# zpelgrims/pota

Hardware: AMD Instinct MI355X
Metric: bidir redistribution Msamples/s at 4K, double-gauss 50mm (higher is better)
Workload: dtype f64

## Files before the change

### include/lentil_hip.h

```cpp
#ifndef LENTIL_HIP_H
#define LENTIL_HIP_H

#include <stddef.h>
#include <stdint.h>

#ifdef __cplusplus
extern "C" {
#endif

#define LENTIL_ABI_VERSION 1

#define LENTIL_OK 0
#define LENTIL_ERR_INVALID (-1)
#define LENTIL_ERR_HIP (-2)
#define LENTIL_ERR_UNSUPPORTED (-3)
#define LENTIL_ERR_NOMEM (-4)

#define LENTIL_THINLENS 0
#define LENTIL_POLYNOMIAL_OPTICS 1
#define LENTIL_UNIT_MM 0
#define LENTIL_UNIT_CM 1
#define LENTIL_UNIT_DM 2
#define LENTIL_UNIT_M 3
#define LENTIL_FILTER_GAUSSIAN 0
// ... 267 lines not shown
  uint64_t first_ray;
  const float *in;
  float *out;
  int32_t *tries;
  double lambda;
  float exposure;
  uint32_t rng_seed;
  uint32_t flags;
} lentil_camera_ray_batch;
int lentil_hip_camera_rays(lentil_hip_ctx *ctx, const lentil_camera_ray_batch *batch);

int lentil_hip_test_y0_intersection(lentil_hip_ctx *ctx, uint64_t n, const double *sensor_shift, double lambda,
                                    double *distance, double *sensor, double *out);
int lentil_hip_test_lt_sample_aperture(lentil_hip_ctx *ctx, uint64_t n, const double *scene,
                                       const double *ap, double lambda, double *sensor,
                                       double *out, double *transmittance);
int lentil_hip_test_trace_bw_po(lentil_hip_ctx *ctx, uint64_t n, const double *target,
                                const int32_t *px, const int32_t *py, const int32_t *attempt,
                                double *sensor_xy, int32_t *ok);
int lentil_hip_test_aperture_sample(lentil_hip_ctx *ctx, uint64_t n, const uint32_t *a,
                                    const uint32_t *b, double *xy);
int lentil_hip_test_xor128_jump(const uint32_t in[4], uint64_t k, uint32_t out[4]);
int lentil_hip_debug_scan_bands(const lentil_params *params, float out[8]);
enum {
  LENTIL_SCAN_DMA2 = 1,
  LENTIL_SCAN_DMA = 2,
  LENTIL_SCAN_DMA_MULTI = 3,
  LENTIL_SCAN_UNIFORM = 4,
  LENTIL_SCAN_UNIFORM_MULTI = 5,
  LENTIL_SCAN_RUNS = 6,
  LENTIL_SCAN_RAGGED = 7
};
int lentil_hip_debug_last_scan(lentil_hip_ctx *ctx, uint32_t out[4]);

#ifdef __cplusplus
}
#endif
#endif
```

### pota_amd/capi.py

```python
import ctypes as C
import os

import numpy as np

from . import _abi

_PKG = os.path.dirname(os.path.abspath(__file__))
LIB_PATH = os.environ.get("LENTIL_HIP_LIB") or os.path.join(_PKG, "liblentil_hip.so")

EXPORTS = [
    "lentil_hip_abi_version", "lentil_hip_create", "lentil_hip_destroy", "lentil_hip_last_error", "lentil_hip_last_redo_note",
    "lentil_hip_set_params", "lentil_hip_set_lens", "lentil_hip_set_bokeh", "lentil_hip_alloc_frame", "lentil_hip_set_camera_motion", "lentil_hip_set_camera_shutter",
    "lentil_hip_upload_visits", "lentil_hip_bind_visits", "lentil_hip_clear_frame",
    "lentil_hip_redistribute", "lentil_hip_resolve", "lentil_hip_sync", "lentil_hip_download_aov",
    "lentil_hip_download_accum", "lentil_hip_download_records", "lentil_hip_accum_buffer", "lentil_hip_stream",
    "lentil_hip_set_closest_exchange", "lentil_hip_zkey_buffer", "lentil_hip_closest_gather",
    "lentil_hip_touched_rows", "lentil_hip_merge_rows", "lentil_hip_resolve_rows",
    "lentil_hip_pack_rows", "lentil_hip_merge_packed_rows", "lentil_hip_compact_rows", "lentil_hip_merge_sparse",
    "lentil_hip_get_counters", "lentil_hip_last_timing", "lentil_hip_last_launches", "lentil_hip_set_draw_log",
    "lentil_hip_batch_model_stats", "lentil_hip_process_stats", "lentil_hip_process_stall_notes", "lentil_hip_set_async", "lentil_hip_pass_totals", "lentil_hip_set_occlusion_probe", "lentil_hip_probe_stats", "lentil_hip_debug_batch_estimate", "lentil_hip_box_probe",
    "lentil_hip_lens_jit_status", "lentil_hip_lens_jit_wait", "lentil_hip_debug_lens_jit_source", "lentil_hip_debug_lens_jit_compile",
    "lentil_hip_download_draw_log", "lentil_hip_test_lt_sample_aperture",
    "lentil_hip_test_trace_bw_po", "lentil_hip_test_aperture_sample", "lentil_hip_debug_scan_bands", "lentil_hip_debug_last_scan",
    "lentil_hip_lens_is_compiled", "lentil_hip_set_lens_mode",
    "lentil_hip_focus_search", "lentil_hip_test_y0_intersection", "lentil_hip_camera_rays",
    "lentil_hip_set_xor128_state", "lentil_hip_get_xor128_state", "lentil_hip_tl_chroma_stats", "lentil_hip_test_xor128_jump",
    "lentil_hip_host_alloc", "lentil_hip_host_free", "lentil_hip_visits_begin", "lentil_hip_visits_append",
    "lentil_hip_visits_wait", "lentil_hip_visits_end",
    "lentil_hip_comm_unique_id", "lentil_hip_comm_init", "lentil_hip_comm_destroy", "lentil_hip_allreduce",
    "lentil_hip_exchange_bands", "lentil_hip_exchange_stats", "lentil_hip_exchange_counts", "lentil_hip_degenerate_stats", "lentil_hip_streams_concurrent",
    "lentil_hip_alloc_crypto", "lentil_hip_upload_crypto", "lentil_hip_bind_crypto", "lentil_hip_download_crypto",
    "lentil_hip_download_crypto_table", "lentil_hip_visits_begin_crypto", "lentil_hip_visits_append_crypto",
]

SCAN_DMA2, SCAN_DMA, SCAN_DMA_MULTI, SCAN_UNIFORM, SCAN_UNIFORM_MULTI, SCAN_RUNS, SCAN_RAGGED = range(1, 8)
SCAN_NAMES = {SCAN_DMA2: "dma2", SCAN_DMA: "dma", SCAN_DMA_MULTI: "dma_multi", SCAN_UNIFORM: "uniform",
              SCAN_UNIFORM_MULTI: "uniform_multi", SCAN_RUNS: "runs", SCAN_RAGGED: "ragged"}

_lib = None


def process_stats():
    lib = load_library()
    n = (C.c_uint64 * 4)()
    rc = lib.lentil_hip_process_stats(n)
    if rc:
        raise RuntimeError("lentil_hip_process_stats: %d" % rc)
    return tuple(int(x) for x in n)


def process_stall_notes():
    lib = load_library()
    buf = C.create_string_buffer(1 << 14)
    lib.lentil_hip_process_stall_notes(buf, 1 << 14)
    return buf.value.decode(errors="replace")

# ... 47 lines not shown
        "lentil_hip_last_error": (C.c_char_p, [vp]),
        "lentil_hip_last_redo_note": (C.c_char_p, [vp]),
        "lentil_hip_set_params": (i, [vp, C.POINTER(_abi.Params)]),
        "lentil_hip_set_lens": (i, [vp, C.POINTER(_abi.LensTable)]),
        "lentil_hip_set_bokeh": (i, [vp, C.POINTER(_abi.BokehTable)]),
        "lentil_hip_alloc_frame": (i, [vp, u32, vp]),
        "lentil_hip_set_camera_motion": (i, [vp, u32, vp]),
        "lentil_hip_set_camera_shutter": (i, [vp, C.c_float, C.c_float]),
        "lentil_hip_upload_visits": (i, [vp, C.POINTER(_abi.Visits)]),
        "lentil_hip_bind_visits": (i, [vp, C.POINTER(_abi.Visits)]),
        "lentil_hip_clear_frame": (i, [vp]),
        "lentil_hip_redistribute": (i, [vp]),
        "lentil_hip_resolve": (i, [vp]),
        "lentil_hip_sync": (i, [vp]),
        "lentil_hip_download_aov": (i, [vp, u32, vp]),
        "lentil_hip_download_accum": (i, [vp, u32, vp, vp]),
        "lentil_hip_download_records": (i, [vp, vp, u64, C.POINTER(u32)]),
        "lentil_hip_accum_buffer": (i, [vp, C.POINTER(vp), C.POINTER(u64)]),
        "lentil_hip_stream": (i, [vp, C.POINTER(vp)]),
        "lentil_hip_set_closest_exchange": (i, [vp, i, u32]),
        "lentil_hip_zkey_buffer": (i, [vp, C.POINTER(vp), C.POINTER(u64)]),
        "lentil_hip_closest_gather": (i, [vp]),
        "lentil_hip_touched_rows": (i, [vp, C.POINTER(C.c_int32), C.POINTER(C.c_int32)]),
        "lentil_hip_merge_rows": (i, [vp, u32, u32, vp, vp]),
        "lentil_hip_pack_rows": (i, [vp, u32, u32, vp]),
        "lentil_hip_merge_packed_rows": (i, [vp, u32, u32, vp, vp]),
        "lentil_hip_compact_rows": (i, [vp, u32, u32, vp, vp, vp, u32, C.POINTER(u32)]),
        "lentil_hip_merge_sparse": (i, [vp, u32, u32, u32, vp, vp, vp]),
        "lentil_hip_resolve_rows": (i, [vp, u32, u32]),
        "lentil_hip_get_counters": (i, [vp, C.POINTER(_abi.Counters)]),
        "lentil_hip_last_timing": (i, [vp, C.POINTER(C.c_float)]),
        "lentil_hip_last_launches": (i, [vp, C.POINTER(C.c_uint32)]),
        "lentil_hip_debug_last_scan": (i, [vp, C.POINTER(C.c_uint32)]),
        "lentil_hip_batch_model_stats": (i, [vp, C.POINTER(C.c_uint64)]),
        "lentil_hip_process_stats": (i, [C.POINTER(C.c_uint64)]),
        "lentil_hip_process_stall_notes": (i, [C.c_char_p, C.c_uint64]),
        "lentil_hip_set_async": (i, [vp, i]),
        "lentil_hip_set_occlusion_probe": (i, [vp, vp, vp, vp]),
        "lentil_hip_probe_stats": (i, [vp, C.POINTER(C.c_uint64)]),
        "lentil_hip_pass_totals": (i, [vp, C.POINTER(_abi.PassTotals), i]),
        "lentil_hip_box_probe": (i, [vp, C.POINTER(C.c_double)]),
        "lentil_hip_lens_jit_status": (i, [vp, C.POINTER(C.c_int), C.POINTER(C.c_double)]),
        "lentil_hip_lens_jit_wait": (i, [vp, C.c_double]),
        "lentil_hip_debug_lens_jit_compile": (i, [vp, i, C.c_char_p, C.c_uint64, C.POINTER(C.c_uint64), C.c_char_p, C.c_uint64,
                                                  C.POINTER(C.c_double), C.POINTER(C.c_uint64)]),
        "lentil_hip_debug_lens_jit_source": (i, [vp, C.c_char_p, C.c_uint64, C.POINTER(C.c_uint64)]),
        "lentil_hip_debug_batch_estimate": (i, [vp, C.c_uint64, vp, C.c_uint32, vp]),
        "lentil_hip_alloc_crypto": (i, [vp, u32, u32]),
        "lentil_hip_upload_crypto": (i, [vp, C.POINTER(_abi.CryptoVisits)]),
        "lentil_hip_bind_crypto": (i, [vp, C.POINTER(_abi.CryptoVisits)]),
        "lentil_hip_download_crypto": (i, [vp, u32, u32, vp, vp]),
        "lentil_hip_visits_begin_crypto": (i, [vp, u32]),
        "lentil_hip_visits_append_crypto": (i, [vp, C.POINTER(_abi.Visits), C.POINTER(_abi.CryptoVisits), C.POINTER(u64)]),
        "lentil_hip_download_crypto_table": (i, [vp, u32, C.POINTER(u32), vp, vp, vp]),
        "lentil_hip_set_draw_log": (i, [vp, u64]),
        "lentil_hip_download_draw_log": (i, [vp, vp, u64, C.POINTER(u64)]),
        "lentil_hip_test_lt_sample_aperture": (i, [vp, u64, vp, vp, C.c_double, vp, vp, vp]),
        "lentil_hip_test_trace_bw_po": (i, [vp, u64, vp, vp, vp, vp, vp, vp]),
        "lentil_hip_test_aperture_sample": (i, [vp, u64, vp, vp, vp]),
        "lentil_hip_lens_is_compiled": (i, [vp]),
        "lentil_hip_set_lens_mode": (i, [vp, i]),
        "lentil_hip_focus_search": (i, [vp, C.c_double, C.c_double, C.POINTER(C.c_double)]),
        "lentil_hip_camera_rays": (i, [vp, C.POINTER(_abi.CameraRayBatch)]),
        "lentil_hip_set_xor128_state": (i, [vp, C.POINTER(C.c_uint32)]),
        "lentil_hip_get_xor128_state": (i, [vp, C.POINTER(C.c_uint32)]),
        "lentil_hip_tl_chroma_stats": (i, [vp, C.POINTER(u64), C.POINTER(u64), C.POINTER(u64)]),
# ... 385 lines not shown

    def set_occlusion_probe(self, fn, user=None, camera_to_world=None):
        self._probe_keep = (np.ascontiguousarray(camera_to_world, np.float32) if camera_to_world is not None else None)
        self._chk(self.lib.lentil_hip_set_occlusion_probe(self.h, fn, user, self._probe_keep.ctypes.data if self._probe_keep is not None else None))

    def probe_stats(self):
        n = (C.c_uint64 * 3)()
        self._chk(self.lib.lentil_hip_probe_stats(self.h, n))
        return tuple(int(x) for x in n)

    def set_async(self, on):
        self._chk(self.lib.lentil_hip_set_async(self.h, 1 if on else 0))

    def pass_totals(self, reset=False):
        t = _abi.PassTotals()
        self._chk(self.lib.lentil_hip_pass_totals(self.h, C.byref(t), 1 if reset else 0))
        return t

    def last_timing(self):
        ms = (C.c_float * 3)()
        self._chk(self.lib.lentil_hip_last_timing(self.h, ms))
        return float(ms[0]), float(ms[1]), float(ms[2])

    def last_launches(self):
        n = (C.c_uint32 * 2)()
        self._chk(self.lib.lentil_hip_last_launches(self.h, n))
        return int(n[0]), int(n[1])

    def last_scan(self):
        n = (C.c_uint32 * 4)()
        self._chk(self.lib.lentil_hip_debug_last_scan(self.h, n))
        return tuple(int(x) for x in n)

    def lens_jit_status(self):
        st, sec = C.c_int(0), C.c_double(0.0)
        self._chk(self.lib.lentil_hip_lens_jit_status(self.h, C.byref(st), C.byref(sec)))
        return int(st.value), float(sec.value)

    def lens_jit_wait(self, timeout_seconds=0.0):
        self._chk(self.lib.lentil_hip_lens_jit_wait(self.h, float(timeout_seconds)))

    def lens_jit_source(self):
        n = C.c_uint64(0)
        self._chk(self.lib.lentil_hip_debug_lens_jit_source(self.h, None, 0, C.byref(n)))
        buf = C.create_string_buffer(int(n.value) + 1)
        self._chk(self.lib.lentil_hip_debug_lens_jit_source(self.h, buf, int(n.value) + 1, None))
        return buf.value.decode()

    def box_probe(self):
        p = (C.c_double * 6)()
        self._chk(self.lib.lentil_hip_box_probe(self.h, p))
        return {"fp64_mul_add_tflops": round(p[0], 2), "shader_clock_mhz_under_fp64": round(p[1], 1), "copy_gbs": round(p[2], 1),
                "read_gbs": round(p[3], 1), "gpu_max_hw_queues": int(p[4]), "compute_units": int(p[5])}

    def batch_model_stats(self):
        n = (C.c_uint64 * 4)()
        self._chk(self.lib.lentil_hip_batch_model_stats(self.h, n))
        return tuple(int(x) for x in n)

    def debug_batch_estimate(self, cs_xyz, samples):
        import numpy as np
        cs = np.ascontiguousarray(cs_xyz, np.float32)
        out = np.zeros((cs.shape[0], 4), np.float32)
        self._chk(self.lib.lentil_hip_debug_batch_estimate(self.h, cs.shape[0], cs.ctypes.data, int(samples), out.ctypes.data))
        return out

# ... 64 lines not shown
```

### pota_amd/csrc/lentil_hip.hip

```cpp
#include <hip/hip_runtime.h>
#include <hip/hip_ext.h>

#include <algorithm>
#include <atomic>
#include <chrono>
#include <cmath>
#include <cstdio>
#include <cstdlib>
#include <cstring>
#include <deque>
#include <mutex>
#include <new>
#include <string>
#include <vector>

#include "lentil_kernels.h"
#include "lentil_closest_replay.h"
#include "lentil_tl_chroma_mgpu.h"
#include "lentil_lens_jit.h"
#include "lentil_camera_rays.h"
#include "generated/embedded_sources.inc"

#define LENTIL_API extern "C" __attribute__((visibility("default")))

// ... 3858 lines not shown
  ms[0] = ms[1] = ms[2] = 0.f;
  HIP_TRY(ctx, hipSetDevice(ctx->device));
  HIP_TRY(ctx, hipStreamSynchronize(ctx->stream));
  if (ctx->timed_draw) {
    HIP_TRY(ctx, hipEventElapsedTime(&ms[0], ctx->ev[0], ctx->ev[1]));
    HIP_TRY(ctx, hipEventElapsedTime(&ms[1], ctx->ev[1], ctx->ev[2]));
    if (ctx->scan_kernel_timed) {
      float k = 0.f;
      if (hipEventElapsedTime(&k, ctx->ev_scan_k[0], ctx->ev_scan_k[1]) == hipSuccess && k > 0.f && k <= ms[0]) {
        ms[1] += ms[0] - k;
        ms[0] = k;
      }
    }
  }
  if (ctx->timed_resolve) HIP_TRY(ctx, hipEventElapsedTime(&ms[2], ctx->ev[3], ctx->ev[4]));
  return LENTIL_OK;
}

LENTIL_API int lentil_hip_last_launches(lentil_hip_ctx *ctx, uint32_t n[2]) {
  CHECK_CTX(ctx);
  if (!n) return fail(ctx, LENTIL_ERR_INVALID, "n is null");
  n[0] = ctx->last_scan_launches;
  n[1] = (uint32_t)ctx->last_rounds;
  return LENTIL_OK;
}

LENTIL_API int lentil_hip_debug_last_scan(lentil_hip_ctx *ctx, uint32_t out[4]) {
  CHECK_CTX(ctx);
  if (!out) return fail(ctx, LENTIL_ERR_INVALID, "out is null");
  for (int i = 0; i < 4; ++i) out[i] = ctx->last_scan[i];
  return LENTIL_OK;
}

static void crypto_log_set_by_caller(lentil_hip_ctx *ctx);
LENTIL_API int lentil_hip_set_draw_log(lentil_hip_ctx *ctx, uint64_t capacity) {
  CHECK_CTX(ctx);
  crypto_log_set_by_caller(ctx);
  HIP_TRY(ctx, hipSetDevice(ctx->device));
  HIP_TRY(ctx, hipStreamSynchronize(ctx->stream));
  (void)hipFree(ctx->d_log);
  ctx->d_log = nullptr;
  ctx->log_cap = 0;
  if (capacity) {
    HIP_TRY(ctx, hipMalloc(&ctx->d_log, capacity * sizeof(lentil_draw_record)));
    ctx->log_cap = capacity;
  }
  return LENTIL_OK;
}

LENTIL_API int lentil_hip_download_draw_log(lentil_hip_ctx *ctx, lentil_draw_record *out, uint64_t capacity,
                                            uint64_t *n_records) {
  CHECK_CTX(ctx);
  if (!n_records) return fail(ctx, LENTIL_ERR_INVALID, "n_records is null");
  DevCounters c;
  HIP_TRY(ctx, hipSetDevice(ctx->device));
  HIP_TRY(ctx, hipMemcpyAsync(&c, ctx->d_ctr + ctx->n_chunks, sizeof(c), hipMemcpyDeviceToHost, ctx->stream));
  HIP_TRY(ctx, hipStreamSynchronize(ctx->stream));
  *n_records = c.log_count;
  uint64_t n = c.log_count < ctx->log_cap ? c.log_count : ctx->log_cap;
  if (n > capacity) n = capacity;
  if (out && n) HIP_TRY(ctx, hipMemcpy(out, ctx->d_log, n * sizeof(lentil_draw_record), hipMemcpyDeviceToHost));
  return LENTIL_OK;
}

template <typename T>
static int dev_copy_in(lentil_hip_ctx *ctx, const T *src, size_t n, T **dst, std::vector<void *> &tmp) {
// ... 363 lines not shown
```

### pota_amd/csrc/lentil_kernels.h

```cpp
#pragma once
#include "lentil_device.h"
#include "lentil_batch_model.h"
#include "generated/lens_registry.h"

using namespace lentil;

struct DevCounters {
  unsigned long long work_count;
  unsigned long long sum_samples;
  unsigned long long redistributed;
  unsigned long long attempted;
  unsigned long long accepted;
  unsigned long long overflow;
  unsigned long long log_count;
  unsigned long long newton_iters;
  unsigned long long tries;
  unsigned long long lane_rounds;
  unsigned long long slow_solves;
  unsigned long long fallback;
  unsigned long long rounds_used;
  unsigned int n_tasks[2];
  unsigned int task_head[2];
  unsigned int n_active[2];
  unsigned int active_head[2];
  unsigned long long pool_used[2];
  unsigned int n_slow[2];
  unsigned int slow_head[2];
  unsigned int waves_started[2], waves_done[2];
  unsigned int accept_done[2];
  unsigned int inv_row_min, row_max_p1;
  unsigned int scan_blocks_done, publishers_done;
  unsigned int n_ranges, range_head;
  unsigned int stuck, tile_next;
  unsigned int degenerate_depth, pad_;
  unsigned int reserved_[8];
  unsigned int accept_started[2];
  unsigned int stuck_info[8];
  unsigned int accept_items_done[2], accept_final[2];
  unsigned int probe_accept_xcc[8], probe_res_xcc[3][8];
  unsigned int probe_snap[1 + 8 + 24 + 2];
};

LD_DEV uint32_t xcc_id() { return (uint32_t)__builtin_amdgcn_s_getreg((3 << 11) | 20) & 7u; }

LD_DEV void flush_row_range(DevCounters *ctr, uint32_t rmin, uint32_t rmax_p1) {
  for (int off = 32; off > 0; off >>= 1) {
    const uint32_t a = __shfl_down(rmin, off), b = __shfl_down(rmax_p1, off);
    rmin = a < rmin ? a : rmin;
    rmax_p1 = b > rmax_p1 ? b : rmax_p1;
  }
  if ((threadIdx.x & 63u) == 0u && rmax_p1) {
    atomicMax(&ctr->inv_row_min, 0x7FFFFFFFu - rmin);
    atomicMax(&ctr->row_max_p1, rmax_p1);
  }
}

struct VisitsDev {
  uint64_t n;
  uint32_t visits_per_pixel, pixels_per_row;
  int32_t pixel_x0, pixel_y0;
  uint32_t pixel_row_stride, n_extra;
  const float4 *rgba, *pos_z, *raydir_time, *volume_ignore, *transmission;
  const float4 *extra[LENTIL_MAX_AOVS - 1];
  const uint32_t *pixel;
  const float *inv_density;
  uint32_t id_base;
  CamMotion cam;
};
// ... 563 lines not shown
  typedef const __attribute__((address_space(1))) void *gptr_t;
  typedef __attribute__((address_space(3))) void *lptr_t;
  __builtin_amdgcn_global_load_lds((gptr_t)(const void *)g, (lptr_t)(void *)lds_wave_base, 16, 0, 2);
}

LD_DEV uint32_t scan_order(const ScanArgs &a, uint32_t t, uint32_t run) {
  if (!a.outside_in) return t;
  const uint32_t n_runs = (uint32_t)((a.tile_end - a.tile_begin + run - 1u) / run);
  const uint32_t k = t / run;
  return ((k & 1u) ? n_runs - 1u - (k >> 1) : (k >> 1)) * run;
}

LD_DEV void wait_vmcnt(uint32_t n) {
#define LENTIL_VMCNT_CASE(N) case N: asm volatile("s_waitcnt vmcnt(" #N ")" ::: "memory"); break;
  switch (n) {
    LENTIL_VMCNT_CASE(0) LENTIL_VMCNT_CASE(1) LENTIL_VMCNT_CASE(2) LENTIL_VMCNT_CASE(3) LENTIL_VMCNT_CASE(4)
    LENTIL_VMCNT_CASE(5) LENTIL_VMCNT_CASE(6) LENTIL_VMCNT_CASE(7) LENTIL_VMCNT_CASE(8) LENTIL_VMCNT_CASE(9)
    LENTIL_VMCNT_CASE(10) LENTIL_VMCNT_CASE(11) LENTIL_VMCNT_CASE(12) LENTIL_VMCNT_CASE(13) LENTIL_VMCNT_CASE(14)
    LENTIL_VMCNT_CASE(15) LENTIL_VMCNT_CASE(16) LENTIL_VMCNT_CASE(17) LENTIL_VMCNT_CASE(18) LENTIL_VMCNT_CASE(19)
    LENTIL_VMCNT_CASE(20) LENTIL_VMCNT_CASE(21) LENTIL_VMCNT_CASE(22) LENTIL_VMCNT_CASE(23) LENTIL_VMCNT_CASE(24)
    LENTIL_VMCNT_CASE(25) LENTIL_VMCNT_CASE(26) LENTIL_VMCNT_CASE(27) LENTIL_VMCNT_CASE(28) LENTIL_VMCNT_CASE(29)
    LENTIL_VMCNT_CASE(30) LENTIL_VMCNT_CASE(31) LENTIL_VMCNT_CASE(32) LENTIL_VMCNT_CASE(33) LENTIL_VMCNT_CASE(34)
    LENTIL_VMCNT_CASE(35) LENTIL_VMCNT_CASE(36) LENTIL_VMCNT_CASE(37) LENTIL_VMCNT_CASE(38) LENTIL_VMCNT_CASE(39)
    LENTIL_VMCNT_CASE(40) LENTIL_VMCNT_CASE(41) LENTIL_VMCNT_CASE(42) LENTIL_VMCNT_CASE(43) LENTIL_VMCNT_CASE(44)
    LENTIL_VMCNT_CASE(45) LENTIL_VMCNT_CASE(46) LENTIL_VMCNT_CASE(47) LENTIL_VMCNT_CASE(48) LENTIL_VMCNT_CASE(49)
    LENTIL_VMCNT_CASE(50) LENTIL_VMCNT_CASE(51) LENTIL_VMCNT_CASE(52) LENTIL_VMCNT_CASE(53) LENTIL_VMCNT_CASE(54)
    LENTIL_VMCNT_CASE(55) LENTIL_VMCNT_CASE(56) LENTIL_VMCNT_CASE(57) LENTIL_VMCNT_CASE(58) LENTIL_VMCNT_CASE(59)
    LENTIL_VMCNT_CASE(60) LENTIL_VMCNT_CASE(61) LENTIL_VMCNT_CASE(62) LENTIL_VMCNT_CASE(63)
    default: asm volatile("s_waitcnt vmcnt(0)" ::: "memory"); break;
  }
#undef LENTIL_VMCNT_CASE
}

__host__ __device__ constexpr uint32_t dma_wave_f4(uint32_t M, uint32_t ring = kDmaRing) { return M * 64u + ring * 192u + 16u; }

template <uint32_t kColBytes = 1024u>
LD_DEV void lds_read_slot(const float4 *slot_lane, float4 &c0, float4 &c1, float4 &c2) {
  typedef float v4f __attribute__((ext_vector_type(4)));
  typedef const __attribute__((address_space(3))) void *lptr_t;
  const uint32_t addr = (uint32_t)(size_t)(lptr_t)(const void *)slot_lane;
  v4f x, y, z;
  asm volatile("ds_read_b128 %0, %3\n\tds_read_b128 %1, %3 offset:%4\n\tds_read_b128 %2, %3 offset:%5\n\ts_waitcnt lgkmcnt(0)"
               : "=&v"(x), "=&v"(y), "=&v"(z)
               : "v"(addr), "n"(kColBytes), "n"(2u * kColBytes)
               : "memory");
  c0 = make_float4(x.x, x.y, x.z, x.w);
  c1 = make_float4(y.x, y.y, y.z, y.w);
  c2 = make_float4(z.x, z.y, z.z, z.w);
}

__global__ __launch_bounds__(256) void scan_dma_kernel(ScanArgs a) {
  LENTIL_TL_SPAN(SPAN_SCAN);
  extern __shared__ float4 smem[];
  const uint32_t lane = threadIdx.x & 63u, wave = threadIdx.x >> 6;
  const VisitsDev &V = a.V;
  const uint32_t M = V.visits_per_pixel;
  const uint32_t R = a.ring >= 2u && a.ring <= 8u ? a.ring : kDmaRing;
  const uint32_t wave_f4 = dma_wave_f4(M, R);
  float4 *srgba = smem + (size_t)wave * wave_f4;
  float4 *ring = srgba + (size_t)M * 64u;
  uint32_t *nskip = reinterpret_cast<uint32_t *>(ring + R * 192u);
  uint2 *qmem = reinterpret_cast<uint2 *>(smem + (size_t)4u * wave_f4);
  WaveQueue wq;
  wq.init(qmem + (size_t)wave * kWaveQueueLds);

  __builtin_amdgcn_s_setprio(3);
// ... 58 lines not shown
      __builtin_amdgcn_fence(__ATOMIC_RELEASE, "wavefront", "local");
      __builtin_amdgcn_wave_barrier();
      __builtin_amdgcn_fence(__ATOMIC_ACQUIRE, "wavefront", "local");
      const uint64_t pix = pix0 + lane;
      const uint32_t skipped = nskip[lane];
      nskip[lane] = 0u;
      if (pix < n_pixels) {
        float4 s = make_float4(0.f, 0.f, 0.f, 0.f);
        for (uint32_t j = 0; j < M; ++j) {
          const float4 c = srgba[lane * M + j];
          s.x += (c.x + 0.0f) * w; s.y += (c.y + 0.0f) * w; s.z += (c.z + 0.0f) * w; s.w += (c.w + 0.0f) * w;
        }
        float ws = 0.f;
        const uint32_t cnt = M - skipped;
        for (uint32_t j = 0; j < cnt; ++j) ws += w;
        const int px = V.pixel_x0 + (int)(pix % V.pixels_per_row);
        const int py = V.pixel_y0 + (int)(pix / V.pixels_per_row) * (int)V.pixel_row_stride;
        const uint64_t lin = (uint64_t)px + (uint64_t)py * xres;
        dir4[lin * 2u] = s;
        dir4[lin * 2u + 1u] = make_float4(ws, 0.f, 0.f, 0.f);
      }
      __builtin_amdgcn_fence(__ATOMIC_RELEASE, "wavefront", "local");
      __builtin_amdgcn_wave_barrier();
      wq.end_tile(a);
    }
    if (lane == 0) tl_add(TL_SCAN_TILES, (uint32_t)(tile4_end - tile4));
  }
  wq.finish(a);
  scan_block_done(a);
}

__host__ __device__ constexpr uint32_t dma2_wave_f4(uint32_t M) { return 2u * M * 64u + 2u * 192u + 16u; }
LD_DEV float4 lds_read_f4(const float4 *p);

LD_DEV void dma2_col(const float4 *ubase, uint32_t lane16, float4 *lds_uniform) {
  typedef const __attribute__((address_space(1))) void *gptr_t;
  typedef __attribute__((address_space(3))) void *lptr_t;
  __builtin_amdgcn_global_load_lds((gptr_t)(const void *)(reinterpret_cast<const char *>(ubase) + lane16), (lptr_t)(void *)lds_uniform, 16, 0, 2);
}
LD_DEV void lds_read_3f4(const float4 *p, float4 &c0, float4 &c1, float4 &c2) {
  typedef float v4f __attribute__((ext_vector_type(4)));
  typedef const __attribute__((address_space(3))) void *lptr_t;
  const uint32_t addr = (uint32_t)(size_t)(lptr_t)(const void *)p;
  v4f x, y, z;
  asm volatile("ds_read_b128 %0, %3\n\tds_read_b128 %1, %3 offset:16\n\tds_read_b128 %2, %3 offset:32\n\ts_waitcnt lgkmcnt(0)"
               : "=&v"(x), "=&v"(y), "=&v"(z)
               : "v"(addr)
               : "memory");
  c0 = make_float4(x.x, x.y, x.z, x.w); c1 = make_float4(y.x, y.y, y.z, y.w); c2 = make_float4(z.x, z.y, z.z, z.w);
}

LD_DEV int coc_below_by_bands(const ScanBands &B, float cz) {
  const bool in0 = cz >= B.in_lo[0] && cz <= B.in_hi[0];
  const bool in1 = cz >= B.in_lo[1] && cz <= B.in_hi[1];
  const bool out0 = cz >= B.out_lo[0] && cz <= B.out_hi[0];
  const bool out1 = cz >= B.out_lo[1] && cz <= B.out_hi[1];
  if (in0 || in1) return 1;
  if (out0 || out1) return 2;
  return 0;
}

__global__ __launch_bounds__(256) void scan_dma2_kernel(ScanArgs a) {
  LENTIL_TL_SPAN(SPAN_SCAN);
  extern __shared__ float4 smem[];
  if (blockIdx.x < a.skip_blocks) { scan_block_done(a); return; }
  const uint32_t lane = threadIdx.x & 63u, wave = (uint32_t)__builtin_amdgcn_readfirstlane((int)(threadIdx.x >> 6));
// ... 2 lines not shown
  const uint32_t wave_f4 = dma2_wave_f4(M);
  float4 *rg = smem + (size_t)wave * wave_f4;
  float4 *ring = rg + (size_t)2u * M * 64u;
  uint32_t *nskip = reinterpret_cast<uint32_t *>(ring + 384u);
  uint2 *qmem = reinterpret_cast<uint2 *>(smem + (size_t)4u * wave_f4);
  WaveQueue wq;
  wq.init(qmem + (size_t)wave * kWaveQueueLds);
  __builtin_amdgcn_s_setprio(3);

  const uint32_t lane16 = lane * 16u;
  const uint32_t TV = 64u * M;
  const uint64_t full_end = (V.n / TV) < a.tile_end ? (V.n / TV) : a.tile_end;
  const float w = 1.0f * a.P.inverse_sample_density;
  float ws_full = 0.f;
  for (uint32_t j = 0; j < M; ++j) ws_full += w;
  float4 *dir4 = reinterpret_cast<float4 *>(a.F.dir);
  const uint32_t xres = a.P.xres;
  const float mz0 = a.P.world_to_camera[0][2], mz1 = a.P.world_to_camera[1][2], mz2 = a.P.world_to_camera[2][2], mz3 = a.P.world_to_camera[3][2];
  float scale = 1.0f;
  if (a.P.unitModel == LENTIL_UNIT_MM) scale = 0.1f;
  else if (a.P.unitModel == LENTIL_UNIT_DM) scale = 10.0f;
  else if (a.P.unitModel == LENTIL_UNIT_M) scale = 100.0f;
  const bool never = a.P.adaptive_sampling && a.P.inverse_sample_density > 0.2f;
  const double inside_lens = a.lens_length * 0.1;
  const bool po = a.P.cameraType == LENTIL_POLYNOMIAL_OPTICS;

  nskip[lane] = 0u;
  auto issue_ring = [&](uint64_t v_group, uint32_t slot) {
    float4 *s = ring + (size_t)slot * 192u;
    dma2_col(V.pos_z + v_group, lane16, s);
    dma2_col(V.volume_ignore + v_group, lane16, s + 64);
    dma2_col(V.transmission + v_group, lane16, s + 128);
  };

  auto do_tile = [&](uint64_t tile, bool has_next, uint64_t next_tile, uint32_t buf, uint32_t par) {
    const uint64_t v0 = tile * TV;
    const uint64_t nv0 = next_tile * TV;
    float4 *srgba = rg + (size_t)buf * M * 64u;
    float4 *nrgba = rg + (size_t)(buf ^ 1u) * M * 64u;
    bool tile_any = false;
    for (uint32_t g = 0; g < M; ++g) {
      if (has_next) asm volatile("s_waitcnt vmcnt(5)" ::: "memory");
      else if (g + 1u < M) asm volatile("s_waitcnt vmcnt(3)" ::: "memory");
      else asm volatile("s_waitcnt vmcnt(0)" ::: "memory");
      const uint32_t slot = (par + g) & 1u;
      float4 pz, vi, tr;
      lds_read_slot(ring + (size_t)slot * 192u + lane, pz, vi, tr);
      if (g + 2u < M) issue_ring(v0 + (uint64_t)(g + 2u) * 64u, slot);
      else if (has_next) issue_ring(nv0 + (uint64_t)(g + 2u - M) * 64u, slot);
      if (has_next) dma2_col(V.rgba + nv0 + (uint64_t)g * 64u, lane16, nrgba + (size_t)g * 64u);
      const float wx = pz.x, wy = pz.y, wz = pz.z, depth = pz.w;
      const bool small = fabsf(wx) < kAiEpsilon && fabsf(wy) < kAiEpsilon && fabsf(wz) < kAiEpsilon;
      const bool far = (depth == kAiInfinite) || small;
      const float cz = (wx * mz0 + wy * mz1 + wz * mz2 + mz3) * scale;
      const int below = coc_below_by_bands(a.bands, cz);
      bool flagged;
      if (__ballot((far && a.P.enable_skydome) || below == 2) == 0ull) {
        bool r = !never && !far;
        if (fmaxf(fmaxf(vi.x, vi.y), vi.z) > 0.0f) r = false;
        if (!a.P.enable_bidir_transmission && fmaxf(fmaxf(tr.x, tr.y), tr.z) > 0.0f) r = false;
        if (vi.w > 0.0f) r = false;
        if (below == 1) r = false;
        if (po && (double)fabsf(cz) < inside_lens) r = false;
        flagged = r;
      } else {
        const uint64_t v = v0 + (uint64_t)g * 64u + lane;
        flagged = visit_redistributes(a.P, a.lens_length, pz, vi, tr, a.P.inverse_sample_density,
                                      [&]() { return V.raydir_time[v]; }, V.cam);
      }
      if (__ballot(flagged)) {
        tile_any = true;
        const uint32_t e = g * 64u + lane;
        const uint64_t v = v0 + e;
        int samples = 0;
        if (flagged) {
          samples = visit_prologue(a.P, a.lens_length, lds_read_f4(srgba + e), pz, V.raydir_time[v], vi, tr, a.P.inverse_sample_density, V.cam).samples;
          srgba[e] = make_float4(0.f, 0.f, 0.f, 0.f);
          atomicAdd(&nskip[e / M], 1u);
        }
        wq.push(flagged, (uint32_t)v, (uint32_t)samples, a);
      }
    }
    typedef float v2f __attribute__((ext_vector_type(2)));
    v2f s01 = {0.f, 0.f}, s23 = {0.f, 0.f};
    const v2f w2 = {w, w};
    const float4 *mine = srgba + (size_t)lane * M;
    uint32_t j = 0;
    for (; j + 3u <= M; j += 3u) {
// ... 5 lines not shown
      p = (v2f){c2.x, c2.y} * w2; s01 += p; p = (v2f){c2.z, c2.w} * w2; s23 += p;
    }
    for (; j < M; ++j) {
      const float4 c0 = lds_read_f4(mine + j);
      v2f p;
      p = (v2f){c0.x, c0.y} * w2; s01 += p; p = (v2f){c0.z, c0.w} * w2; s23 += p;
    }
    float ws = ws_full;
    if (tile_any) {
      asm volatile("s_waitcnt vmcnt(0)" ::: "memory");
      __builtin_amdgcn_fence(__ATOMIC_RELEASE, "wavefront", "local");
      __builtin_amdgcn_wave_barrier();
      __builtin_amdgcn_fence(__ATOMIC_ACQUIRE, "wavefront", "local");
      const uint32_t skipped = nskip[lane];
      nskip[lane] = 0u;
      ws = 0.f;
      for (uint32_t q = 0; q < M - skipped; ++q) ws += w;
    }
    {
      const uint32_t pix = (uint32_t)(tile * 64u) + lane;
      const uint32_t row = __umulhi(pix, a.ppr_magic) >> a.ppr_shift;
      const uint32_t col = pix - row * V.pixels_per_row;
      const int px = V.pixel_x0 + (int)col;
      const int py = V.pixel_y0 + (int)row * (int)V.pixel_row_stride;
      const uint64_t lin = (uint64_t)px + (uint64_t)py * xres;
      dir4[lin * 2u] = make_float4(s01.x, s01.y, s23.x, s23.y);
      dir4[lin * 2u + 1u] = make_float4(ws, 0.f, 0.f, 0.f);
    }
    if (tile_any) {
      __builtin_amdgcn_fence(__ATOMIC_RELEASE, "wavefront", "local");
      __builtin_amdgcn_wave_barrier();
      wq.end_tile(a);
    }
  };

  const uint64_t n_full = full_end > a.tile_begin ? full_end - a.tile_begin : 0ull;
  const uint32_t n_runs = (uint32_t)((n_full + 3u) / 4u);
  const uint32_t W = (gridDim.x - a.skip_blocks) * 4u;
  const uint32_t R = n_runs / W;
  const uint32_t n_lvl = (R >= 2u ? 1u : 0u) + (R >= 4u ? 1u : 0u) + (R >= 8u ? 1u : 0u) + (R >= 16u ? 1u : 0u);
  const uint32_t lb1 = (R >> 1) * W, lb2 = lb1 + (R >> 2) * W, lb3 = lb2 + (R >> 3) * W, lb4 = lb3 + (R >> 4) * W;
  auto run_first = [&](uint32_t r) { return a.tile_begin + (uint64_t)(a.outside_in ? ((r & 1u) ? n_runs - 1u - (r >> 1) : (r >> 1)) : r) * 4u; };
  auto run_len = [&](uint64_t first) { return (uint32_t)(full_end - first < 4u ? full_end - first : 4u); };
  uint32_t buf = 0, par = 0;
  while (true) {
    uint32_t t = 0;
    if (lane == 0) t = atomicAdd(&a.ctr->tile_next, 1u);
    t = (uint32_t)__builtin_amdgcn_readfirstlane(t);
    uint32_t r, runs_left, stride;
    if (t < n_lvl * W) {
      const uint32_t l = t / W;
      r = (l == 0u ? 0u : (l == 1u ? lb1 : (l == 2u ? lb2 : lb3))) + (t - l * W);
      runs_left = R >> (l + 1u);
      stride = W;
    } else {
      r = lb4 + (t - n_lvl * W);
      runs_left = 1u;
      stride = 0u;
      if (r >= n_runs) break;
    }
    uint64_t tile = run_first(r);
    uint32_t left = run_len(tile);
    {
      const uint64_t v0 = tile * TV;
      for (uint32_t g = 0; g < M; ++g) dma2_col(V.rgba + v0 + (uint64_t)g * 64u, lane16, rg + (size_t)buf * M * 64u + (size_t)g * 64u);
      issue_ring(v0, par);
      if (M > 1u) issue_ring(v0 + 64u, par ^ 1u);
      asm volatile("s_waitcnt vmcnt(0)" ::: "memory");
    }
    while (true) {
      bool has_next = false;
      uint64_t next_tile = tile;
      uint32_t next_left = 0;
      if (left > 1u) { has_next = true; next_tile = tile + 1u; next_left = left - 1u; }
      else if (runs_left > 1u) {
        has_next = true;
        next_tile = run_first(r + stride);
        next_left = run_len(next_tile);
      }
      do_tile(tile, has_next, next_tile, buf, par);
      if (lane == 0) tl_add(TL_SCAN_TILES, 1u);
      buf ^= 1u;
      par = (par + M) & 1u;
      if (left == 1u) { r += stride; --runs_left; }
      if (!has_next) break;
      tile = next_tile; left = next_left;
    }
  }
  if (a.tile_end > full_end && blockIdx.x == a.skip_blocks && wave == 0) {
    const uint64_t tile = full_end;
    const uint64_t n_pixels = V.n / M;
    const uint64_t pix = tile * 64u + lane;
    asm volatile("s_waitcnt vmcnt(0)" ::: "memory");
    float4 s = make_float4(0.f, 0.f, 0.f, 0.f);
    float ws = 0.f;
    for (uint32_t j = 0; j < M; ++j) {
      const uint64_t v = pix * M + j;
      const bool valid = pix < n_pixels;
      bool flagged = false;
      int samples = 0;
      float4 c = make_float4(0.f, 0.f, 0.f, 0.f);
      if (valid) {
        const float4 pz = V.pos_z[v], vi = V.volume_ignore[v], tr = V.transmission[v];
        c = V.rgba[v];
        flagged = visit_redistributes(a.P, a.lens_length, pz, vi, tr, a.P.inverse_sample_density, [&]() { return V.raydir_time[v]; }, V.cam);
        if (flagged) samples = visit_prologue(a.P, a.lens_length, c, pz, V.raydir_time[v], vi, tr, a.P.inverse_sample_density, V.cam).samples;
      }
      if (valid && !flagged) { s.x += c.x * w; s.y += c.y * w; s.z += c.z * w; s.w += c.w * w; ws += w; }
      wq.push(flagged, (uint32_t)v, (uint32_t)samples, a);
    }
    if (pix < n_pixels) {
      const int px = V.pixel_x0 + (int)(pix % V.pixels_per_row);
      const int py = V.pixel_y0 + (int)(pix / V.pixels_per_row) * (int)V.pixel_row_stride;
      const uint64_t lin = (uint64_t)px + (uint64_t)py * xres;
      dir4[lin * 2u] = s;
      dir4[lin * 2u + 1u] = make_float4(ws, 0.f, 0.f, 0.f);
    }
    wq.end_tile(a);
  }
  asm volatile("s_waitcnt vmcnt(0)" ::: "memory");
  wq.finish(a);
  scan_block_done(a);
}

LD_DEV float4 lds_read_f4(const float4 *p) {
  typedef float v4f __attribute__((ext_vector_type(4)));
  typedef const __attribute__((address_space(3))) void *lptr_t;
  const uint32_t addr = (uint32_t)(size_t)(lptr_t)(const void *)p;
  v4f x;
  asm volatile("ds_read_b128 %0, %1\n\ts_waitcnt lgkmcnt(0)" : "=&v"(x) : "v"(addr) : "memory");
  return make_float4(x.x, x.y, x.z, x.w);
}
LD_DEV void lds_read_4f4(const float4 *p, float4 c[4]) {
  typedef float v4f __attribute__((ext_vector_type(4)));
  typedef const __attribute__((address_space(3))) void *lptr_t;
  const uint32_t addr = (uint32_t)(size_t)(lptr_t)(const void *)p;
  v4f x, y, z, w;
  asm volatile("ds_read_b128 %0, %4\n\tds_read_b128 %1, %4 offset:16\n\tds_read_b128 %2, %4 offset:32\n\tds_read_b128 %3, %4 offset:48\n\t"
               "s_waitcnt lgkmcnt(0)"
               : "=&v"(x), "=&v"(y), "=&v"(z), "=&v"(w)
               : "v"(addr)
               : "memory");
  c[0] = make_float4(x.x, x.y, x.z, x.w); c[1] = make_float4(y.x, y.y, y.z, y.w);
  c[2] = make_float4(z.x, z.y, z.z, z.w); c[3] = make_float4(w.x, w.y, w.z, w.w);
}
LD_DEV float4 global_read_f4_untracked(const float4 *p) {
  typedef float v4f __attribute__((ext_vector_type(4)));
  v4f x;
  asm volatile("global_load_dwordx4 %0, %1, off\n\ts_waitcnt vmcnt(0)" : "=&v"(x) : "v"(p) : "memory");
  return make_float4(x.x, x.y, x.z, x.w);
}
constexpr uint32_t kDmaMultiRun = 16;
constexpr uint32_t kDmaMultiCol = 65;
// ... 3081 lines not shown
```

Before: 40740.

## Add lean scan mode loading only pos_z, fetching other attributes on candidates

Measured after the change: 41840, median of 6. 1.03x the previous value.

```diff
diff --git a/include/lentil_hip.h b/include/lentil_hip.h
--- a/include/lentil_hip.h
+++ b/include/lentil_hip.h
@@ -323,6 +323,7 @@
   LENTIL_SCAN_RAGGED = 7
 };
 int lentil_hip_debug_last_scan(lentil_hip_ctx *ctx, uint32_t out[4]);
+int lentil_hip_debug_scan_extra_groups(lentil_hip_ctx *ctx, uint64_t *out);
 
 #ifdef __cplusplus
 }
diff --git a/pota_amd/capi.py b/pota_amd/capi.py
--- a/pota_amd/capi.py
+++ b/pota_amd/capi.py
@@ -21,7 +21,7 @@
     "lentil_hip_batch_model_stats", "lentil_hip_process_stats", "lentil_hip_process_stall_notes", "lentil_hip_set_async", "lentil_hip_pass_totals", "lentil_hip_set_occlusion_probe", "lentil_hip_probe_stats", "lentil_hip_debug_batch_estimate", "lentil_hip_box_probe",
     "lentil_hip_lens_jit_status", "lentil_hip_lens_jit_wait", "lentil_hip_debug_lens_jit_source", "lentil_hip_debug_lens_jit_compile",
     "lentil_hip_download_draw_log", "lentil_hip_test_lt_sample_aperture",
-    "lentil_hip_test_trace_bw_po", "lentil_hip_test_aperture_sample", "lentil_hip_debug_scan_bands", "lentil_hip_debug_last_scan",
+    "lentil_hip_test_trace_bw_po", "lentil_hip_test_aperture_sample", "lentil_hip_debug_scan_bands", "lentil_hip_debug_last_scan", "lentil_hip_debug_scan_extra_groups",
     "lentil_hip_lens_is_compiled", "lentil_hip_set_lens_mode",
     "lentil_hip_focus_search", "lentil_hip_test_y0_intersection", "lentil_hip_camera_rays",
     "lentil_hip_set_xor128_state", "lentil_hip_get_xor128_state", "lentil_hip_tl_chroma_stats", "lentil_hip_test_xor128_jump",
@@ -135,6 +135,7 @@
         "lentil_hip_last_timing": (i, [vp, C.POINTER(C.c_float)]),
         "lentil_hip_last_launches": (i, [vp, C.POINTER(C.c_uint32)]),
         "lentil_hip_debug_last_scan": (i, [vp, C.POINTER(C.c_uint32)]),
+        "lentil_hip_debug_scan_extra_groups": (i, [vp, C.POINTER(C.c_uint64)]),
         "lentil_hip_batch_model_stats": (i, [vp, C.POINTER(C.c_uint64)]),
         "lentil_hip_process_stats": (i, [C.POINTER(C.c_uint64)]),
         "lentil_hip_process_stall_notes": (i, [C.c_char_p, C.c_uint64]),
@@ -586,6 +587,11 @@
         self._chk(self.lib.lentil_hip_debug_last_scan(self.h, n))
         return tuple(int(x) for x in n)
 
+    def scan_extra_groups(self):
+        n = C.c_uint64(0)
+        self._chk(self.lib.lentil_hip_debug_scan_extra_groups(self.h, C.byref(n)))
+        return int(n.value)
+
     def lens_jit_status(self):
         st, sec = C.c_int(0), C.c_double(0.0)
         self._chk(self.lib.lentil_hip_lens_jit_status(self.h, C.byref(st), C.byref(sec)))
diff --git a/pota_amd/csrc/lentil_hip.hip b/pota_amd/csrc/lentil_hip.hip
--- a/pota_amd/csrc/lentil_hip.hip
+++ b/pota_amd/csrc/lentil_hip.hip
@@ -3914,6 +3914,22 @@
   return LENTIL_OK;
 }
 
+LENTIL_API int lentil_hip_debug_scan_extra_groups(lentil_hip_ctx *ctx, uint64_t *out) {
+  CHECK_CTX(ctx);
+  if (!out) return fail(ctx, LENTIL_ERR_INVALID, "out is null");
+  std::vector<DevCounters> c((size_t)ctx->n_chunks);
+  if (ctx->h_ctr_valid && ctx->h_ctr.size() == c.size()) {
+    c = ctx->h_ctr;
+  } else {
+    HIP_TRY(ctx, hipSetDevice(ctx->device));
+    HIP_TRY(ctx, hipStreamSynchronize(ctx->stream));
+    HIP_TRY(ctx, hipMemcpy(c.data(), ctx->d_ctr, sizeof(DevCounters) * c.size(), hipMemcpyDeviceToHost));
+  }
+  *out = 0;
+  for (const DevCounters &k : c) *out += k.scan_extra_groups;
+  return LENTIL_OK;
+}
+
 static void crypto_log_set_by_caller(lentil_hip_ctx *ctx);
 LENTIL_API int lentil_hip_set_draw_log(lentil_hip_ctx *ctx, uint64_t capacity) {
   CHECK_CTX(ctx);
diff --git a/pota_amd/csrc/lentil_kernels.h b/pota_amd/csrc/lentil_kernels.h
--- a/pota_amd/csrc/lentil_kernels.h
+++ b/pota_amd/csrc/lentil_kernels.h
@@ -33,7 +33,8 @@
   unsigned int n_ranges, range_head;
   unsigned int stuck, tile_next;
   unsigned int degenerate_depth, pad_;
-  unsigned int reserved_[8];
+  unsigned int scan_extra_groups;
+  unsigned int reserved_[7];
   unsigned int accept_started[2];
   unsigned int stuck_info[8];
   unsigned int accept_items_done[2], accept_final[2];
@@ -663,6 +664,16 @@
 #undef LENTIL_VMCNT_CASE
 }
 
+LD_DEV void wait_vmcnt_12(uint32_t n) {
+#define LENTIL_VMCNT_CASE(N) case N: asm volatile("s_waitcnt vmcnt(" #N ")" ::: "memory"); break;
+  switch (n) {
+    LENTIL_VMCNT_CASE(1) LENTIL_VMCNT_CASE(2) LENTIL_VMCNT_CASE(3) LENTIL_VMCNT_CASE(4) LENTIL_VMCNT_CASE(5) LENTIL_VMCNT_CASE(6)
+    LENTIL_VMCNT_CASE(7) LENTIL_VMCNT_CASE(8) LENTIL_VMCNT_CASE(9) LENTIL_VMCNT_CASE(10) LENTIL_VMCNT_CASE(11)
+    default: asm volatile("s_waitcnt vmcnt(0)" ::: "memory"); break;
+  }
+#undef LENTIL_VMCNT_CASE
+}
+
 __host__ __device__ constexpr uint32_t dma_wave_f4(uint32_t M, uint32_t ring = kDmaRing) { return M * 64u + ring * 192u + 16u; }
 
 template <uint32_t kColBytes = 1024u>
@@ -787,6 +798,16 @@
 
 __host__ __device__ constexpr uint32_t dma2_wave_f4(uint32_t M) { return 2u * M * 64u + 2u * 192u + 16u; }
 LD_DEV float4 lds_read_f4(const float4 *p);
+constexpr uint32_t kDma2LeanSlots = 6;
+LD_DEV void global_read_2f4_untracked(const float4 *p0, const float4 *p1, float4 &c0, float4 &c1) {
+  typedef float v4f __attribute__((ext_vector_type(4)));
+  v4f x, y;
+  asm volatile("global_load_dwordx4 %0, %2, off\n\tglobal_load_dwordx4 %1, %3, off\n\ts_waitcnt vmcnt(0)"
+               : "=&v"(x), "=&v"(y)
+               : "v"(p0), "v"(p1)
+               : "memory");
+  c0 = make_float4(x.x, x.y, x.z, x.w); c1 = make_float4(y.x, y.y, y.z, y.w);
+}
 
 LD_DEV void dma2_col(const float4 *ubase, uint32_t lane16, float4 *lds_uniform) {
   typedef const __attribute__((address_space(1))) void *gptr_t;
@@ -855,28 +876,57 @@
     dma2_col(V.volume_ignore + v_group, lane16, s + 64);
     dma2_col(V.transmission + v_group, lane16, s + 128);
   };
-
-  auto do_tile = [&](uint64_t tile, bool has_next, uint64_t next_tile, uint32_t buf, uint32_t par) {
+  auto issue_lean = [&](uint64_t v_group, uint32_t slot) { dma2_col(V.pos_z + v_group, lane16, ring + (size_t)slot * 64u); };
+  const uint32_t S = M < kDma2LeanSlots ? M : kDma2LeanSlots;
+  auto is_candidate = [&](bool far, int below, float cz) {
+    if (never) return false;
+    if (far) return a.P.enable_skydome != 0;
+    return below != 1 && !(po && (double)fabsf(cz) < inside_lens);
+  };
+  uint32_t extra_groups = 0;
+
+  auto do_tile = [&](uint64_t tile, bool has_next, uint64_t next_tile, uint32_t buf, bool dense, uint32_t &slot) {
     const uint64_t v0 = tile * TV;
     const uint64_t nv0 = next_tile * TV;
     float4 *srgba = rg + (size_t)buf * M * 64u;
     float4 *nrgba = rg + (size_t)(buf ^ 1u) * M * 64u;
     bool tile_any = false;
+    uint32_t cand_groups = 0;
     for (uint32_t g = 0; g < M; ++g) {
-      if (has_next) asm volatile("s_waitcnt vmcnt(5)" ::: "memory");
-      else if (g + 1u < M) asm volatile("s_waitcnt vmcnt(3)" ::: "memory");
-      else asm volatile("s_waitcnt vmcnt(0)" ::: "memory");
-      const uint32_t slot = (par + g) & 1u;
       float4 pz, vi, tr;
-      lds_read_slot(ring + (size_t)slot * 192u + lane, pz, vi, tr);
-      if (g + 2u < M) issue_ring(v0 + (uint64_t)(g + 2u) * 64u, slot);
-      else if (has_next) issue_ring(nv0 + (uint64_t)(g + 2u - M) * 64u, slot);
+      if (dense) {
+        if (has_next) asm volatile("s_waitcnt vmcnt(5)" ::: "memory");
+        else if (g + 1u < M) asm volatile("s_waitcnt vmcnt(3)" ::: "memory");
+        else asm volatile("s_waitcnt vmcnt(0)" ::: "memory");
+        lds_read_slot(ring + (size_t)slot * 192u + lane, pz, vi, tr);
+        if (g + 2u < M) issue_ring(v0 + (uint64_t)(g + 2u) * 64u, slot);
+        else if (has_next) issue_ring(nv0 + (uint64_t)(g + 2u - M) * 64u, slot);
+        slot ^= 1u;
+      } else {
+        if (has_next) { if (S == kDma2LeanSlots) asm volatile("s_waitcnt vmcnt(11)" ::: "memory"); else wait_vmcnt_12(2u * S - 1u); }
+        else wait_vmcnt_12((M - 1u - g) < (S - 1u) ? (M - 1u - g) : (S - 1u));
+        pz = lds_read_f4(ring + (size_t)slot * 64u + lane);
+        vi = make_float4(0.f, 0.f, 0.f, 0.f);
+        tr = make_float4(0.f, 0.f, 0.f, 0.f);
+        if (g + S < M) issue_lean(v0 + (uint64_t)(g + S) * 64u, slot);
+        else if (has_next) issue_lean(nv0 + (uint64_t)(g + S - M) * 64u, slot);
+        slot = slot + 1u == S ? 0u : slot + 1u;
+      }
       if (has_next) dma2_col(V.rgba + nv0 + (uint64_t)g * 64u, lane16, nrgba + (size_t)g * 64u);
       const float wx = pz.x, wy = pz.y, wz = pz.z, depth = pz.w;
       const bool small = fabsf(wx) < kAiEpsilon && fabsf(wy) < kAiEpsilon && fabsf(wz) < kAiEpsilon;
       const bool far = (depth == kAiInfinite) || small;
       const float cz = (wx * mz0 + wy * mz1 + wz * mz2 + mz3) * scale;
       const int below = coc_below_by_bands(a.bands, cz);
+      const bool candidate = is_candidate(far, below, cz);
+      if (__ballot(candidate) != 0ull) {
+        ++cand_groups;
+        if (!dense) {
+          ++extra_groups;
+          if (candidate) global_read_2f4_untracked(V.volume_ignore + v0 + (uint64_t)g * 64u + lane, V.transmission + v0 + (uint64_t)g * 64u + lane, vi, tr);
+        }
+      }
+      if (dense) ++extra_groups;
       bool flagged;
       if (__ballot((far && a.P.enable_skydome) || below == 2) == 0ull) {
         bool r = !never && !far;
@@ -948,6 +998,12 @@
       __builtin_amdgcn_wave_barrier();
       wq.end_tile(a);
     }
+    return cand_groups;
+  };
+  auto fill_ring = [&](uint64_t tile, bool dense) {
+    const uint64_t v0 = tile * TV;
+    if (dense) { issue_ring(v0, 0u); issue_ring(v0 + 64u, 1u); }
+    else for (uint32_t l = 0; l < S; ++l) issue_lean(v0 + (uint64_t)l * 64u, l);
   };
 
   const uint64_t n_full = full_end > a.tile_begin ? full_end - a.tile_begin : 0ull;
@@ -958,7 +1014,8 @@
   const uint32_t lb1 = (R >> 1) * W, lb2 = lb1 + (R >> 2) * W, lb3 = lb2 + (R >> 3) * W, lb4 = lb3 + (R >> 4) * W;
   auto run_first = [&](uint32_t r) { return a.tile_begin + (uint64_t)(a.outside_in ? ((r & 1u) ? n_runs - 1u - (r >> 1) : (r >> 1)) : r) * 4u; };
   auto run_len = [&](uint64_t first) { return (uint32_t)(full_end - first < 4u ? full_end - first : 4u); };
-  uint32_t buf = 0, par = 0;
+  uint32_t buf = 0, slot = 0;
+  bool dense = false;
   while (true) {
     uint32_t t = 0;
     if (lane == 0) t = atomicAdd(&a.ctr->tile_next, 1u);
@@ -980,8 +1037,8 @@
     {
       const uint64_t v0 = tile * TV;
       for (uint32_t g = 0; g < M; ++g) dma2_col(V.rgba + v0 + (uint64_t)g * 64u, lane16, rg + (size_t)buf * M * 64u + (size_t)g * 64u);
-      issue_ring(v0, par);
-      if (M > 1u) issue_ring(v0 + 64u, par ^ 1u);
+      slot = 0u;
+      fill_ring(tile, dense);
       asm volatile("s_waitcnt vmcnt(0)" ::: "memory");
     }
     while (true) {
@@ -994,10 +1051,19 @@
         next_tile = run_first(r + stride);
         next_left = run_len(next_tile);
       }
-      do_tile(tile, has_next, next_tile, buf, par);
+      const uint32_t cand_groups = do_tile(tile, has_next, next_tile, buf, dense, slot);
       if (lane == 0) tl_add(TL_SCAN_TILES, 1u);
       buf ^= 1u;
-      par = (par + M) & 1u;
+      const bool want_dense = cand_groups >= 2u;
+      if (want_dense != dense) {
+        dense = want_dense;
+        if (has_next) {
+          asm volatile("s_waitcnt vmcnt(0)" ::: "memory");
+          slot = 0u;
+          fill_ring(next_tile, dense);
+          asm volatile("s_waitcnt vmcnt(0)" ::: "memory");
+        }
+      }
       if (left == 1u) { r += stride; --runs_left; }
       if (!has_next) break;
       tile = next_tile; left = next_left;
@@ -1016,8 +1082,17 @@
       bool flagged = false;
       int samples = 0;
       float4 c = make_float4(0.f, 0.f, 0.f, 0.f);
+      float4 pz = make_float4(0.f, 0.f, 0.f, 0.f), vi = pz, tr = pz;
+      bool candidate = false;
       if (valid) {
-        const float4 pz = V.pos_z[v], vi = V.volume_ignore[v], tr = V.transmission[v];
+        pz = V.pos_z[v];
+        const bool small = fabsf(pz.x) < kAiEpsilon && fabsf(pz.y) < kAiEpsilon && fabsf(pz.z) < kAiEpsilon;
+        const float cz = (pz.x * mz0 + pz.y * mz1 + pz.z * mz2 + mz3) * scale;
+        candidate = is_candidate((pz.w == kAiInfinite) || small, coc_below_by_bands(a.bands, cz), cz);
+      }
+      if (__ballot(candidate) != 0ull) ++extra_groups;
+      if (candidate) { vi = V.volume_ignore[v]; tr = V.transmission[v]; }
+      if (valid) {
         c = V.rgba[v];
         flagged = visit_redistributes(a.P, a.lens_length, pz, vi, tr, a.P.inverse_sample_density, [&]() { return V.raydir_time[v]; }, V.cam);
         if (flagged) samples = visit_prologue(a.P, a.lens_length, c, pz, V.raydir_time[v], vi, tr, a.P.inverse_sample_density, V.cam).samples;
@@ -1035,6 +1110,7 @@
     wq.end_tile(a);
   }
   asm volatile("s_waitcnt vmcnt(0)" ::: "memory");
+  if (lane == 0 && extra_groups) atomicAdd(&a.ctr->scan_extra_groups, extra_groups);
   wq.finish(a);
   scan_block_done(a);
 }
```
